# gau-nernst/pytorch-models

Measured on AMD Instinct MI355X. Metric: ViT-B/16 images/s & Whisper-base audio-sec/s (BASELINE.json metric; value / unit / ms_per_step = the ViT-B/16 leg of configs[1], the Whisper-base leg of configs[2] is the "whisper" object), higher is better.
Workload: dtype bf16; 1 GPU; ViT-B/16 bf16 forward, batch=256 per GPU, 224x224 (BASELINE configs[1]); per_gpu_batch=256, global_batch=256, parallelism=dp1, collective=none

## Files before the change

### include/pm_mi355x.h

```cpp
#ifndef PM_MI355X_H
#define PM_MI355X_H
#include <stdint.h>
#ifdef __cplusplus
extern "C" {
#endif

#define PM_ABI_VERSION 1

enum { PM_OK = 0, PM_EINVAL = 1, PM_EUNSUPPORTED = 2, PM_ELAUNCH = 3, PM_EALIGN = 4 };
enum { PM_BF16 = 0, PM_F32 = 1 };
enum { PM_ACT_NONE = 0, PM_ACT_GELU = 1, PM_ACT_GELU_TANH = 2, PM_ACT_RELU = 3, PM_ACT_SILU = 4 };

int pm_abi_version(void);
const char* pm_strerror(int code);

int pm_linear_bf16(const void* x, int64_t ldx, const void* w, int64_t ldw, const float* bias,
                   const void* resid, int64_t ldr, int resid_dtype, void* y, int64_t ldy, int y_dtype,
                   int64_t M, int64_t N, int64_t K, int act, void* stream);

int pm_linear_bf16_ex(const void* x, int64_t ldx, int64_t x_rows_per_batch, int64_t x_batch_stride, const void* w,
                      int64_t ldw, const float* bias, const void* resid, int64_t ldr, int resid_dtype,
                      int64_t resid_period, void* y, int64_t ldy, int y_dtype, int64_t M, int64_t N, int64_t K, int act,
                      void* stream);

// ... 195 lines not shown
                           int64_t k_stride_t, const void* v, int64_t v_stride_b, int64_t v_stride_t, void* o,
                           int64_t o_stride_b, int64_t o_stride_t, int64_t B, int64_t H, int64_t Lq, int64_t Lk, void* stream);

int pm_mixer_token_mix_bf16(const void* x, const float* stats, const float* gamma, const float* beta, const void* w1,
                            const float* b1, const void* w2, const float* b2, void* y, float* row_out, int64_t N, int64_t T,
                            int64_t Dt, int64_t C, void* stream);
int pm_mixer_token_mix_supported(int64_t T, int64_t Dt, int64_t C);

int pm_row_stats(const void* x, int64_t ldx, int x_dtype, float* stats, int64_t M, int64_t C, float eps, void* stream);

int pm_ln_mean(const void* x, int x_dtype, const float* stats, const float* gamma, const float* beta, void* y, int y_dtype,
               int64_t N, int64_t T, int64_t C, void* stream);

int pm_transpose_add_f32(const float* x, const float* resid, float* y, int64_t ldy, int64_t N, int64_t R, int64_t Cc, void* stream);

int pm_conv1d_f32(const float* x, int64_t x_batch_stride, const float* w, const float* bias, const float* resid, float* y,
                  int64_t B, int64_t Tin, int64_t Cin, int64_t Cout, int64_t k, int64_t stride, int64_t left, int64_t right,
                  int zero_pad, int elu, int64_t up, int64_t trim, int64_t Tout, void* stream);
int pm_conv1d_f32_supported(int64_t Tin, int64_t Cin, int64_t Cout, int64_t k, int64_t stride, int64_t left, int64_t right,
                            int zero_pad, int64_t up);

int pm_lstm_f32(const float* x, const float* const* w_ih, const float* const* w_hh, const float* const* bias, int64_t n_layers,
                float* work, float* y, int flags, int64_t B, int64_t T, int64_t H, void* stream);
int64_t pm_lstm_workspace_floats(int64_t B, int64_t T, int64_t H);

int pm_rvq_encode_f32(const float* z, const float* codebooks, const float* norms, int64_t* codes, int64_t M, int64_t n_q,
                      int64_t dim, int64_t codebook_size, void* stream);
int pm_rvq_decode_f32(const int64_t* codes, int64_t stride_b, int64_t stride_q, int64_t stride_t, const float* codebooks,
                      float* out, int64_t B, int64_t T, int64_t n_q, int64_t dim, int64_t codebook_size, void* stream);

int pm_groupnorm1_f32(float* x, const float* gamma, const float* beta, const float* resid, double* work, int64_t B, int64_t n,
                      int64_t C, float eps, void* stream);
int64_t pm_groupnorm1_workspace_doubles(int64_t B, int64_t n);

int pm_encodec_scale_f32(const float* x, float* scale, int64_t B, int64_t C, int64_t T, void* stream);
int pm_scale_clips_f32(const float* x, const float* scale, float* y, int64_t B, int64_t n, int divide, void* stream);

int pm_t5_dec_embed(const int64_t* tok, int64_t ldtok, const void* emb, float* x, int64_t B, int64_t d, int64_t V, void* stream);
int pm_t5_dec_self_fused(const float* x, int64_t d, const float* gamma, float eps, const void* w_qkv, void* kcache, void* vcache,
                         int64_t Tmax, const int32_t* pos_ptr, const float* lut, float* att, int64_t B, int64_t H, void* stream);
int pm_t5_dec_rms_qkv(const float* x, int64_t d, const float* gamma, float eps, const void* w_qkv, float* q, void* kcache,
                      void* vcache, int64_t Tmax, const int32_t* pos_ptr, int64_t B, int64_t H, void* stream);
int pm_t5_dec_self_attention(const float* q, const void* kcache, const void* vcache, int64_t Tmax, const int32_t* pos_ptr,
                             const float* lut, float* att, int64_t B, int64_t H, void* stream);
int pm_t5_dec_cross_fused(const float* x, int64_t d, const float* gamma, float eps, const void* w_q, const void* cross_kv,
                          int64_t S, const int32_t* src_len, float* att, int64_t B, int64_t H, void* stream);
int pm_t5_dec_geglu(const float* x, int64_t d, const float* gamma, float eps, const void* w_wv, float* h, int64_t ldh, int64_t B,
                    int64_t F, void* stream);
int pm_t5_dec_next_token(const float* ws_val, const int32_t* ws_idx, int64_t n_tiles, int32_t* pos_ptr, const int64_t* prompt,
                         int64_t P, int64_t* tokens, int64_t Ttot, int64_t pad_id, int64_t eos_id, int32_t* finished,
                         int64_t* out_lengths, const void* emb, float* x, int64_t d, int64_t V, int32_t* ticket,
                         const float* logits_step, float* logits_all, int64_t B, void* stream);

#ifdef __cplusplus
}
#endif
#endif
```

### pytorch-models_amd/pytorch_models/_hip/__init__.py

```python
from __future__ import annotations

import ctypes
import os
import re
from ctypes import c_char_p, c_float, c_int, c_int64, c_void_p

_HERE = os.path.dirname(os.path.abspath(__file__))
REPO_PKG_ROOT = os.path.dirname(os.path.dirname(_HERE))
LIB_PATH = os.environ.get("PM_MI355X_LIB") or os.path.join(REPO_PKG_ROOT, "csrc", "build", "libpm_mi355x.so")
HEADER_PATH = os.path.join(os.path.dirname(REPO_PKG_ROOT), "include", "pm_mi355x.h")

PM_BF16, PM_F32 = 0, 1
ACT = dict(none=0, gelu=1, approximate_gelu=2, relu=3, silu=4)

_p, _i, _l, _f = c_void_p, c_int, c_int64, c_float
SIGNATURES = {
    "pm_abi_version": ([], c_int),
    "pm_strerror": ([_i], c_char_p),
    "pm_linear_bf16": ([_p, _l, _p, _l, _p, _p, _l, _i, _p, _l, _i, _l, _l, _l, _i, _p], c_int),
    "pm_linear_bf16_ex": ([_p, _l, _l, _l, _p, _l, _p, _p, _l, _i, _l, _p, _l, _i, _l, _l, _l, _i, _p], c_int),
    "pm_linear_bf16_ln": ([_p, _l, _l, _l, _p, _l, _p, _p, _l, _i, _l, _p, _l, _i, _l, _l, _l, _i, _p, _p, _p, _p], c_int),
    "pm_linear_f32": ([_p, _l, _l, _l, _p, _l, _p, _p, _l, _l, _p, _l, _l, _l, _l, _i, _p], c_int),
    "pm_attention_generic_f32": ([_p, _l, _l, _p, _l, _l, _p, _l, _l, _p, _l, _l, _l, _l, _l, _l, _l, _i, _p, _l, _l, _l, _p], c_int),
    "pm_linear_bf16_ws": ([_p, _l, _l, _l, _p, _l, _p, _p, _l, _i, _l, _p, _l, _i, _l, _l, _l, _i, _p, _p, _p, _p, _l, _p], c_int),
# ... 22 lines not shown
    "pm_dec_whisper_rules": ([_p, _l, _l, _p, _l, _p, _l, _l, _l, _l, _l, _p, _l, _p, _l, _l, _p], c_int),
    "pm_dec_sample_topk": ([_p, _l, _l, _l, ctypes.c_uint64, _p, _p, _l, _p, _p, _l, _p, _p, _p, _l, _p, _l, _p], c_int),
    "pm_dec_next_token": ([_p, _p, _l, _p, _p, _l, _p, _p, _l, _p, _p, _p, _p, _l, _l, _p, _l, _p], c_int),
    "pm_layernorm": ([_p, _l, _i, _p, _p, _f, _p, _l, _i, _l, _l, _p], c_int),
    "pm_layernorm_ex": ([_p, _l, _i, _p, _p, _f, _i, _p, _l, _i, _p, _l, _i, _l, _l, _p], c_int),
    "pm_rmsnorm": ([_p, _l, _i, _p, _f, _p, _l, _i, _l, _l, _p], c_int),
    "pm_geglu": ([_p, _l, _p, _l, _l, _l, _p], c_int),
    "pm_w2v_stem0_scratch_floats": ([_l, _l], c_int64),
    "pm_w2v_stem0": ([_p, _p, _p, _i, _p, _p, _f, _p, _p, _p, _l, _l, _l, _l, _l, _p], c_int),
    "pm_group_windows": ([_p, _l, _i, _p, _l, _l, _l, _l, _l, _l, _l, _p], c_int),
    "pm_grouped_conv_supported": ([_l, _l], c_int),
    "pm_grouped_conv_bf16": ([_p, _p, _p, _p, _l, _p, _l, _l, _l, _l, _l, _l, _l, _l, _l, _i, _p], c_int),
    "pm_avgpool_time2": ([_p, _p, _l, _l, _l, _p], c_int),
    "pm_attention_bf16": ([_p, _l, _l, _p, _l, _l, _p, _l, _l, _p, _l, _l, _l, _l, _l, _l, _i, _p], c_int),
    "pm_attention_bias_bf16": ([_p, _l, _l, _p, _l, _l, _p, _l, _l, _p, _l, _l, _l, _l, _l, _l, _i, _p, _l, _l, _l, _p], c_int),
    "pm_attention_generic_bf16": ([_p, _l, _l, _p, _l, _l, _p, _l, _l, _p, _l, _l, _l, _l, _l, _l, _l, _i, _p, _l, _l, _l, _p], c_int),
    "pm_vit_tokens": ([_p, _p, _p, _p, _p, _p, _l, _l, _l, _l, _l, _p], c_int),
    "pm_vit_tokens_generic": ([_p, _p, _l, _p, _p, _p, _p, _l, _l, _l, _l, _l, _p], c_int),
    "pm_dwconv7_ln": ([_p, _i, _p, _p, _p, _p, _f, _p, _l, _i, _l, _l, _l, _l, _p], c_int),
    "pm_ln_space_to_depth": ([_p, _l, _i, _p, _p, _f, _p, _l, _i, _l, _l, _l, _l, _p], c_int),
    "pm_convnext_stem": ([_p, _p, _p, _p, _p, _f, _p, _l, _i, _l, _l, _l, _l, _p], c_int),
    "pm_mean_ln": ([_p, _l, _i, _p, _p, _f, _p, _i, _l, _l, _l, _p], c_int),
    "pm_window_attention_bf16": ([_p, _p, _p, _l, _p, _l, _p, _l, _l, _l, _l, _l, _i, _p], c_int),
    "pm_dwconv3_bn_act": ([_p, _i, _p, _p, _p, _p, _p, _p, _i, _l, _l, _l, _l, _i, _p], c_int),
    "pm_se_gate": ([_p, _l, _l, _p, _p, _p, _p, _p, _l, _l, _l, _p], c_int),
    "pm_maxvit_stem": ([_p, _p, _p, _p, _l, _i, _l, _l, _l, _l, _p], c_int),
    "pm_im2col3x3_nhwc": ([_p, _i, _p, _l, _i, _l, _l, _l, _l, _p], c_int),
    "pm_avgpool2x2_nhwc": ([_p, _i, _p, _i, _l, _l, _l, _l, _p], c_int),
    "pm_conv_bf16": ([_p, _l, _l, _l, _l, _p, _p, _p, _p, _l, _l, _l, _i, _p], c_int),
    "pm_resnet_stem": ([_p, _p, _p, _p, _p, _l, _l, _l, _p], c_int),
    "pm_attention_hd32_bf16": ([_p, _l, _l, _p, _l, _l, _p, _l, _l, _p, _l, _l, _l, _l, _l, _l, _p], c_int),
    "pm_mixer_token_mix_bf16": ([_p, _p, _p, _p, _p, _p, _p, _p, _p, _p, _l, _l, _l, _l, _p], c_int),
    "pm_mixer_token_mix_supported": ([_l, _l, _l], c_int),
    "pm_row_stats": ([_p, _l, _i, _p, _l, _l, _f, _p], c_int),
    "pm_ln_mean": ([_p, _i, _p, _p, _p, _p, _i, _l, _l, _l, _p], c_int),
    "pm_transpose_add_f32": ([_p, _p, _p, _l, _l, _l, _l, _p], c_int),
    "pm_conv1d_f32": ([_p, _l, _p, _p, _p, _p, _l, _l, _l, _l, _l, _l, _l, _l, _i, _i, _l, _l, _l, _p], c_int),
    "pm_conv1d_f32_supported": ([_l, _l, _l, _l, _l, _l, _l, _i, _l], c_int),
    "pm_lstm_f32": ([_p, _p, _p, _p, _l, _p, _p, _i, _l, _l, _l, _p], c_int),
    "pm_lstm_workspace_floats": ([_l, _l, _l], c_int64),
    "pm_rvq_encode_f32": ([_p, _p, _p, _p, _l, _l, _l, _l, _p], c_int),
    "pm_rvq_decode_f32": ([_p, _l, _l, _l, _p, _p, _l, _l, _l, _l, _l, _p], c_int),
    "pm_groupnorm1_f32": ([_p, _p, _p, _p, _p, _l, _l, _l, _f, _p], c_int),
    "pm_groupnorm1_workspace_doubles": ([_l, _l], c_int64),
    "pm_encodec_scale_f32": ([_p, _p, _l, _l, _l, _p], c_int),
    "pm_scale_clips_f32": ([_p, _p, _p, _l, _l, _i, _p], c_int),
    "pm_t5_dec_embed": ([_p, _l, _p, _p, _l, _l, _l, _p], c_int),
    "pm_t5_dec_self_fused": ([_p, _l, _p, _f, _p, _p, _p, _l, _p, _p, _p, _l, _l, _p], c_int),
    "pm_t5_dec_rms_qkv": ([_p, _l, _p, _f, _p, _p, _p, _p, _l, _p, _l, _l, _p], c_int),
    "pm_t5_dec_self_attention": ([_p, _p, _p, _l, _p, _p, _p, _l, _l, _p], c_int),
    "pm_t5_dec_cross_fused": ([_p, _l, _p, _f, _p, _p, _l, _p, _p, _l, _l, _p], c_int),
    "pm_t5_dec_geglu": ([_p, _l, _p, _f, _p, _p, _l, _l, _l, _p], c_int),
    "pm_t5_dec_next_token": ([_p, _p, _l, _p, _p, _l, _p, _l, _l, _l, _p, _p, _p, _p, _l, _l, _p, _p, _p, _l, _p], c_int),
}

EXPERIMENT_SIGNATURES = {
    "pm_dec_attention_fused_v2": ([_p, _l, _p, _p, _f, _p, _p, _p, _p, _l, _l, _l, _p, _l, _l, _p, _l, _l, _i, _p], c_int),
    "pm_dec_layers": ([_p, _l, _l, _l, _l, _l, _l, _l, _i, _l, _p, _p, _p, _p, _l, _p, _p, _p, _p, _p], c_int),
    "pm_dec_layers_grid": ([], c_int),
    "pm_gemm8ph_bench": ([_p, _l, _p, _l, _p, _l, _l, _l, _l, _p], c_int),
}


class DecLayer(ctypes.Structure):
    _fields_ = [(n, c_void_p) for n in (
        "sa_g", "sa_b", "w_qkv", "b_qkv", "kc", "vc", "w_so", "b_so", "ca_g", "ca_b", "w_q", "b_q", "cross_kv", "w_co", "b_co",
        "mlp_g", "mlp_b", "w1", "b1", "w2", "b2")] + [(n, c_float) for n in ("sa_eps", "ca_eps", "mlp_eps", "reserved_")]


_lib = None


def header_functions() -> list[str]:
    src = open(HEADER_PATH).read()
    src = re.sub(r"/\*.*?\*/", "", src, flags=re.S)
    return sorted(set(re.findall(r"\b(pm_[a-z0-9_]+)\s*\(", src)))


def lib() -> ctypes.CDLL:
    global _lib
    if _lib is None:
        if not os.path.exists(LIB_PATH):
            raise RuntimeError(
                f"{LIB_PATH} is missing: the MI355X HIP library has not been built "
                "(run `make -C pytorch-models_amd/csrc` or `python -c 'import __graft_entry__ as g; g.build()'`). "
                "This package has no CPU or eager fallback."
            )
        L = ctypes.CDLL(LIB_PATH)
        for name, (argtypes, restype) in SIGNATURES.items():
            fn = getattr(L, name)
            fn.argtypes = argtypes
            fn.restype = restype
        for name, (argtypes, restype) in EXPERIMENT_SIGNATURES.items():
            if hasattr(L, name):
                fn = getattr(L, name)
                fn.argtypes = argtypes
                fn.restype = restype
        if L.pm_abi_version() != 1:
            raise RuntimeError(f"libpm_mi355x ABI {L.pm_abi_version()} != binding ABI 1: rebuild the library")
        _lib = L
    return _lib


def has_experiments() -> bool:
    return hasattr(lib(), "pm_dec_layers")

# ... 5 lines not shown
```

### pytorch-models_amd/pytorch_models/_hip/ops.py

```python
from __future__ import annotations

import os

import torch
from torch import Tensor

from . import ACT, PM_BF16, PM_F32, check, lib


_raw_stream = getattr(torch._C, "_cuda_getCurrentRawStream", None)
_cur_device = getattr(torch._C, "_cuda_getDevice", None)


def _stream() -> int:
    if _raw_stream is not None and _cur_device is not None:
        return _raw_stream(_cur_device())
    return torch.cuda.current_stream().cuda_stream


def _current_device_index() -> int:
    return _cur_device() if _cur_device is not None else torch.cuda.current_device()


def check_devices(*ts) -> None:
# ... 1009 lines not shown
    _f32c(codebooks, "rvq_decode: codebooks")
    B, n_q, T = codes.shape
    Q, N, D = codebooks.shape
    _need(1 <= n_q <= Q, f"rvq_decode: {n_q} code streams for {Q} codebooks")
    out = torch.empty((B, T, D), dtype=torch.float32, device=codes.device)
    rc = _launch("rvq_decode_f32", (0.0, float(out.numel() * 4 * (n_q + 1))), lambda: lib().pm_rvq_decode_f32(
        codes.data_ptr(), codes.stride(0), codes.stride(1), codes.stride(2), codebooks.data_ptr(), out.data_ptr(), B, T, n_q, D, N, _stream()))
    check(rc, f"pm_rvq_decode_f32(B={B}, T={T}, n_q={n_q})")
    return out


def groupnorm1_(x: Tensor, gamma: Tensor, beta: Tensor, eps: float, resid: Tensor | None = None) -> Tensor:
    _cuda(x, gamma, beta, resid)
    _need(x.dim() == 3, "groupnorm1_: x must be (B, T, C)")
    _f32c(x, "groupnorm1_: x")
    B, T, C = x.shape
    _f32vec(gamma, C, "groupnorm1_: gamma")
    _f32vec(beta, C, "groupnorm1_: beta")
    if resid is not None:
        _need(resid.shape == x.shape, "groupnorm1_: resid must have x's shape")
        _f32c(resid, "groupnorm1_: resid")
    _need(B <= 65535 and T >= 1, "groupnorm1_: at most 65535 clips, at least one frame")
    work = torch.empty((lib().pm_groupnorm1_workspace_doubles(B, T * C),), dtype=torch.float64, device=x.device)
    rc = _launch("groupnorm1_f32", (0.0, float(x.numel() * 12)), lambda: lib().pm_groupnorm1_f32(
        x.data_ptr(), gamma.data_ptr(), beta.data_ptr(), resid.data_ptr() if resid is not None else None, work.data_ptr(), B, T * C, C,
        float(eps), _stream()))
    check(rc, f"pm_groupnorm1_f32(B={B}, T={T}, C={C})")
    return x


def encodec_scale(x: Tensor) -> Tensor:
    _cuda(x)
    _need(x.dim() == 3, "encodec_scale: x must be (B, C, T)")
    _f32c(x, "encodec_scale: x")
    B, C, T = x.shape
    _need(T >= 1 and C >= 1, "encodec_scale: empty clip")
    out = torch.empty((B, 1, 1), dtype=torch.float32, device=x.device)
    rc = _launch("encodec_scale_f32", (0.0, float(x.numel() * 4)), lambda: lib().pm_encodec_scale_f32(x.data_ptr(), out.data_ptr(), B, C, T, _stream()))
    check(rc, f"pm_encodec_scale_f32(B={B}, C={C}, T={T})")
    return out


def scale_clips(x: Tensor, scale: Tensor, divide: bool) -> Tensor:
    _cuda(x, scale)
    _f32c(x, "scale_clips: x")
    _f32c(scale, "scale_clips: scale")
    B = x.shape[0]
    _need(x.dim() >= 2 and scale.numel() == B and B <= 65535 and x.numel() > 0, "scale_clips: one scale per clip, at most 65535 clips")
    out = torch.empty_like(x)
    rc = _launch("scale_clips_f32", (0.0, float(x.numel() * 8)), lambda: lib().pm_scale_clips_f32(
        x.data_ptr(), scale.data_ptr(), out.data_ptr(), B, x.numel() // B, int(divide), _stream()))
    check(rc, "pm_scale_clips_f32")
    return out
```

### pytorch-models_amd/pytorch_models/image/vit.py

```python
from __future__ import annotations

from functools import partial

import torch
import torch.nn.functional as F
from torch import Tensor, nn

from .. import _cpu
from .._hip import ops
from ..transformer import MHA, MLP, Encoder, LayerNorm, _f32, _fused_mlp, _wb, derived


class ClassTokenPooling(nn.Module):
    def forward(self, x: Tensor) -> Tensor:
        return x[:, 0]


class GlobalAveragePooling(nn.Module):
    def forward(self, x: Tensor) -> Tensor:
        return x.mean(1)


class MHAPooling(nn.Module):

# ... 30 lines not shown
        super().__init__()
        self.patch_embed = nn.Conv2d(3, d_model, patch_size, patch_size)
        self.cls_token = nn.Parameter(torch.zeros(1, 1, d_model)) if cls_token else None
        self.pe = nn.Parameter(torch.zeros(1, (img_size // patch_size) ** 2, d_model))
        self.layers = Encoder(n_layers, d_model, n_heads=n_heads, dropout=dropout, norm_eps=self.norm_eps)
        self.layers.pm_streams = 2
        self.norm = LayerNorm(d_model, self.norm_eps)
        poolers = dict(
            cls_token=ClassTokenPooling,
            gap=GlobalAveragePooling,
            mha=partial(MHAPooling, d_model, n_heads, norm_eps=self.norm_eps),
        )
        self.pooler = poolers[pool_type]()

    def tokens(self, imgs: Tensor) -> Tensor:
        if _cpu.on_cpu(imgs, self.patch_embed.weight):
            return _cpu.vit_tokens(self, imgs)
        if self.patch_embed.weight.dtype == torch.float32:
            return self._tokens_f32(imgs)
        pw = self.patch_embed.weight
        if pw.shape[2] == 16:
            w2d = pw.view(pw.shape[0], -1)
        else:
            def pad():
                k = 3 * pw.shape[2] * pw.shape[3]
                w = torch.zeros(pw.shape[0], (k + 63) // 64 * 64, dtype=pw.dtype, device=pw.device)
                w[:, :k] = pw.detach().reshape(pw.shape[0], -1)
                return w

            w2d = derived(self, "w2d_pad", (pw,), pad)
        cls = None if self.cls_token is None else _f32(self, "cls", self.cls_token).view(-1)
        return ops.vit_tokens(imgs.float().contiguous(), w2d, _f32(self, "pb", self.patch_embed.bias),
                              _f32(self, "pe", self.pe).view(-1, pw.shape[0]), cls, pw.shape[2])

    def _tokens_f32(self, imgs: Tensor) -> Tensor:
        w = self.patch_embed.weight
        d, _, P, _ = w.shape
        N, _, H, W = imgs.shape
        gh, gw = H // P, W // P
        cols = imgs.float().unfold(2, P, P).unfold(3, P, P).permute(0, 2, 3, 1, 4, 5).reshape(N * gh * gw, 3 * P * P)
        pe = self.pe.float().view(-1, d)
        if pe.shape[0] != gh * gw:
            raise ValueError(f"ViT: pe holds {pe.shape[0]} positions, the image has {gh * gw} patches; call resize_pe first")
        y = ops.linear_f32(cols, w.view(d, -1), self.patch_embed.bias, resid=pe.contiguous(), resid_period=gh * gw).view(N, gh * gw, d)
        if self.cls_token is not None:
            y = torch.cat([self.cls_token.float().expand(N, 1, d), y], 1)
        return y

    def forward(self, imgs: Tensor) -> Tensor:
        n_tok = self.pe.shape[1] + (self.cls_token is not None)
        parts = None
        if imgs.dim() == 4 and imgs.is_cuda and self.patch_embed.weight.dtype == torch.bfloat16:
            parts = self.layers.split_sizes(imgs.shape[0], n_tok, torch.bfloat16, imgs.device)
        if parts is None:
            out = self.layers(self.tokens(imgs))
        else:
            out = self.layers(producers=[lambda lo=lo, hi=hi: self.tokens(imgs[lo:hi]) for lo, hi in parts], device=imgs.device)
        io = self.patch_embed.weight.dtype
        if isinstance(self.pooler, ClassTokenPooling):
            return self.norm(out[:, 0], io)
        if out.device.type == "cpu":
            return self.pooler(self.norm(out))
        return self.pooler(self.norm(out)).to(io)

    @torch.no_grad()
    def resize_pe(self, size: int, interpolation_mode: str = "bicubic") -> None:
        g_old = int(self.pe.shape[1] ** 0.5)
        g_new = size // self.patch_embed.weight.shape[2]
        grid = self.pe.float().unflatten(1, (g_old, g_old)).permute(0, 3, 1, 2)
        grid = F.interpolate(grid, (g_new, g_new), mode=interpolation_mode)
        self.pe = nn.Parameter(grid.permute(0, 2, 3, 1).flatten(1, 2).to(self.pe.dtype))

    def load_flax_ckpt(self, ckpt, *, big_vision: bool = False, prefix: str = "") -> None:
        from ..converters import load_flax_vit

        left = load_flax_vit(self, ckpt, big_vision=big_vision, prefix=prefix)
        if left:
            print(left)

    def load_facebook_state_dict(self, state_dict) -> None:
        from ..converters import load_facebook_vit

        print(load_facebook_vit(self, state_dict))

    @staticmethod
    def _parse(model_tag: str, default_weights: str):
        tag, weights = model_tag.split("_") if "_" in model_tag else (model_tag, default_weights)
        size, patch = tag.split("/")
        return tag, weights, _SIZES[size], int(patch)

    @staticmethod
    def from_google(model_tag: str, *, pretrained: bool = False, **kwargs) -> "ViT":
        _, weights, (n_layers, d_model, n_heads), patch = ViT._parse(model_tag, "augreg")
        extra = dict(cls_token=False, pool_type="mha") if weights == "siglip" else {}
        m = ViT(n_layers, d_model, n_heads, patch, **extra, **kwargs)
        if pretrained:
            if weights not in ("augreg", "siglip"):
                raise ValueError(f"Unsupported weights={weights}")
            _no_download("ViT.from_google")
        return m

    @staticmethod
    def from_facebook(model_tag: str, *, pretrained: bool = False, **kwargs) -> "ViT":
        _, weights, (n_layers, d_model, n_heads), patch = ViT._parse(model_tag, "deit3")
        if weights in ("deit3", "dino"):
            kwargs.setdefault("img_size", 224)
        elif weights == "dinov2":
            kwargs.setdefault("img_size", 518)
        else:
            raise ValueError(f"Unsupported {weights}")
        m = ViT(n_layers, d_model, n_heads, patch, **kwargs)
        if pretrained:
            _no_download("ViT.from_facebook")
# ... 26 lines not shown
```

### pytorch-models_amd/pytorch_models/transformer.py

```python
from __future__ import annotations

import os

import torch
from torch import Tensor, nn

from . import _cpu
from ._hip import ops

_ACTS = {
    "gelu": lambda: nn.GELU(),
    "approximate_gelu": lambda: nn.GELU(approximate="tanh"),
    "relu": lambda: nn.ReLU(inplace=True),
    "silu": lambda: nn.SiLU(),
}


def _sig(ts) -> tuple:
    return tuple((t.data_ptr(), 0 if t.is_inference() else t._version, t.dtype, t.device) for t in ts if t is not None)


def derived(module: nn.Module, key: str, params, build):
    store = module.__dict__.setdefault("_pm_derived", {})
    sig = _sig(params)
# ... 89 lines not shown
        return y.view(*x.shape[:-1], self.out_features)


class MHA(nn.Module):
    def __init__(
        self,
        d_model: int,
        n_heads: int | None = None,
        head_dim: int | None = None,
        bias: bool = True,
        dropout: float = 0.0,
    ) -> None:
        if n_heads is None and head_dim is None:
            head_dim = 64
        if head_dim is None:
            head_dim = d_model // n_heads
        if n_heads is None:
            n_heads = d_model // head_dim
        super().__init__()
        inner = n_heads * head_dim
        self.q_proj = Linear(d_model, inner, bias)
        self.k_proj = Linear(d_model, inner, bias)
        self.v_proj = Linear(d_model, inner, bias)
        self.out_proj = Linear(inner, d_model, bias)
        self.n_heads = n_heads
        self.head_dim = head_dim
        self.dropout = dropout

    def _pack(self, names: str):
        mods = [getattr(self, f"{n}_proj") for n in names]
        params = [m.weight for m in mods] + [m.bias for m in mods]

        def build():
            w = torch.cat([m.weight.detach() for m in mods], 0).to(torch.bfloat16).contiguous()
            b = None if mods[0].bias is None else torch.cat([m.bias.detach().float() for m in mods], 0).contiguous()
            return w, b

        return derived(self, "pack_" + names, params, build)

    def _pack32(self, names: str):
        mods = [getattr(self, f"{n}_proj") for n in names]
        params = [m.weight for m in mods] + [m.bias for m in mods]

        def build():
            w = torch.cat([m.weight.detach().float() for m in mods], 0).contiguous()
            b = None if mods[0].bias is None else torch.cat([m.bias.detach().float() for m in mods], 0).contiguous()
            return w, b

        return derived(self, "pack32_" + names, params, build)

    def _pack_ln(self, norm: "LayerNorm"):
        w, b = self._pack("qkv")
        return derived(self, "pack_qkv_ln", (w, b, norm.weight, norm.bias), lambda: _fold_ln(w, b, norm))

    def forward(
        self,
        q: Tensor,
        k: Tensor | None = None,
        v: Tensor | None = None,
        attn_bias: Tensor | None = None,
        causal: bool = False,
    ) -> Tensor:
        return self.attend(q, k, v, attn_bias, causal)

    def attend(self, q, k=None, v=None, attn_bias=None, causal=False, residual: Tensor | None = None) -> Tensor:
        if _cpu.on_cpu(q, self.q_proj.weight):
            return _cpu.mha(self, q, k, v, attn_bias, causal, residual)
        _require_bf16(q, self.q_proj.weight, "MHA")
        if self.head_dim % 2 or self.head_dim > 128 or (self.head_dim % 4 and self.head_dim > 64):
            raise NotImplementedError(f"MHA: head_dim {self.head_dim} is not covered by the gfx950 attention kernels (% 4 up to 128, % 2 up to 64)")
        if self.training and self.dropout > 0.0:
            raise NotImplementedError("MHA: inference only (attention dropout is not implemented)")
        H, inner = self.n_heads, self.n_heads * self.head_dim
        Lq = q.shape[-2]
        if _is32(self.q_proj.weight):
            return self._attend_f32(q, k, v, attn_bias, causal, residual)
        io_dtype = q.dtype
        q = _xb(q)
        k = None if k is None else _xb(k)
        v = None if v is None else _xb(v)
        if k is None and v is None:
            lead = q.shape[:-2]
            w, b = self._pack("qkv")
            qkv = ops.linear(q.reshape(-1, q.shape[-1]), w, b).view(-1, Lq, 3 * inner)
            qh, kh, vh = qkv[..., :inner], qkv[..., inner : 2 * inner], qkv[..., 2 * inner :]
        else:
            k = q if k is None else k
            Lk = k.shape[-2]
            lead = torch.broadcast_shapes(q.shape[:-2], k.shape[:-2])
            qh = self.q_proj(q)
            if v is None or v is k:
                w, b = self._pack("kv")
                kv = ops.linear(k.reshape(-1, k.shape[-1]), w, b).view(*k.shape[:-1], 2 * inner)
                kh, vh = kv[..., :inner], kv[..., inner:]
            else:
                kh, vh = self.k_proj(k), self.v_proj(v)
            qh = qh.expand(*lead, Lq, inner).reshape(-1, Lq, inner)
            kh = kh.expand(*lead, Lk, inner).reshape(-1, Lk, inner)
            vh = vh.expand(*lead, Lk, inner).reshape(-1, Lk, inner)
        bias4 = None if attn_bias is None else _bias4(attn_bias, lead, Lq, kh.shape[1])
        o = ops.attention(qh, kh, vh, H, causal, bias4)
        res2 = None if residual is None else residual.reshape(-1, residual.shape[-1])
        y = ops.linear(o.view(-1, inner), _wb(self.out_proj, "w", self.out_proj.weight), _f32(self.out_proj, "b", self.out_proj.bias),
                       resid=res2, out_dtype=io_dtype)
        return y.view(*lead, Lq, y.shape[-1])

# ... 151 lines not shown
        n_heads: int | None = None,
        head_dim: int | None = None,
        bias: bool = True,
        mlp_ratio: float = 4.0,
        dropout: float = 0.0,
        act: str = "gelu",
        pre_norm: bool = True,
        norm_eps: float = 1e-5,
    ) -> None:
        super().__init__(d_model, n_heads, head_dim, False, bias, mlp_ratio, dropout, act, pre_norm, norm_eps)

    def forward(self, x: Tensor) -> Tensor:
        return DecoderLayer.forward(self, x, None)

    def chain_ok(self, x: Tensor) -> bool:
        sa, mlp = self.sa, self.mlp
        if not (self.pre_norm and type(sa).forward is MHA.forward and type(mlp).forward is MLP.forward and x.is_cuda
                and x.dtype == torch.bfloat16 and sa.q_proj.weight.dtype == torch.bfloat16 and not self.training):
            return False
        M, d = x.numel() // x.shape[-1], x.shape[-1]
        inner, hid = sa.n_heads * sa.head_dim, mlp.linear1.out_features
        if sa.head_dim % 8 or sa.head_dim > 128 or mlp.act_name not in ("gelu",):
            return False
        return (ops.linear_ln_supported(M, d, inner, "none", True) and ops.linear_ln_supported(M, d, hid, "none", True)
                and ops.linear_ln_supported(M, 3 * inner, d, "none", False)
                and ops.linear_ln_supported(M, hid, d, mlp.act_name, False))

    def forward_chain(self, x: Tensor, stats: Tensor | None, next_eps: float | None):
        sa, mlp = self.sa, self.mlp
        lead, d = x.shape[:-1], x.shape[-1]
        H, inner = sa.n_heads, sa.n_heads * sa.head_dim
        x2 = x.reshape(-1, d)
        if stats is None:
            w, b = sa._pack("qkv")
            qkv = ops.linear(self.sa_norm(x2), w, b)
        else:
            wl, s, c = sa._pack_ln(self.sa_norm)
            qkv = ops.linear(x2, wl, c, ln_stats=stats, ln_s=s)
        qkv = qkv.view(-1, x.shape[-2], 3 * inner)
        o = ops.attention(qkv[..., :inner], qkv[..., inner : 2 * inner], qkv[..., 2 * inner :], H, False, None)
        x2, rows = ops.linear(o.view(-1, inner), sa.out_proj.weight, _f32(sa.out_proj, "b", sa.out_proj.bias), resid=x2,
                              want_row_stats=True)
        st = ops.ln_stats_finalize(rows, d, self.mlp_norm.eps)
        l1, l2 = mlp.linear1, mlp.linear2
        wl, s, c = derived(mlp, "l1_ln", (l1.weight, l1.bias, self.mlp_norm.weight, self.mlp_norm.bias),
                           lambda: _fold_ln(l1.weight, l1.bias, self.mlp_norm))
        h = ops.linear(x2, wl, c, act=mlp.act_name, ln_stats=st, ln_s=s)
        if next_eps is None:
            return ops.linear(h, l2.weight, _f32(l2, "b", l2.bias), resid=x2).view(*lead, d), None
        x2, rows = ops.linear(h, l2.weight, _f32(l2, "b", l2.bias), resid=x2, want_row_stats=True)
        return x2.view(*lead, d), ops.ln_stats_finalize(rows, d, next_eps)


class Encoder(nn.Sequential):
    def __init__(
        self,
        n_layers: int,
        d_model: int,
        n_heads: int | None = None,
        head_dim: int | None = None,
        bias: bool = True,
        mlp_ratio: float = 4.0,
        dropout: float = 0.0,
        act: str = "gelu",
        pre_norm: bool = True,
        norm_eps: float = 1e-5,
    ) -> None:
        super().__init__(*[
            EncoderLayer(d_model, n_heads, head_dim, bias, mlp_ratio, dropout, act, pre_norm, norm_eps)
            for _ in range(n_layers)
        ])

    def forward(self, x: Tensor | None = None, *, producers=None, device: torch.device | None = None) -> Tensor:
        layers = list(self)
        fold = os.environ.get("PM_LN_FOLD", "1") != "0"

        def plan(t: Tensor):
            return [fold and isinstance(l, EncoderLayer) and type(l).forward is EncoderLayer.forward and l.chain_ok(t) for l in layers]

        def step(i: int, ok, t: Tensor, stats):
            if not ok[i]:
                return layers[i](t), None
            nxt = layers[i + 1].sa_norm.eps if i + 1 < len(layers) and ok[i + 1] else None
            return layers[i].forward_chain(t, stats, nxt)

        halves = self._two_streams(x) if producers is None else None
        if halves is not None and any(plan(h) != plan(halves[0]) for h in halves[1:]):
            halves = None
        if halves is None and producers is None:
            ok, stats = plan(x), None
            for i in range(len(layers)):
                x, stats = step(i, ok, x, stats)
            return x
        n_parts = len(halves) if producers is None else len(producers)
        device = halves[0].device if producers is None else device
        cur = torch.cuda.current_stream(device)
        streams = [cur] + [_side_stream(device, k) for k in range(1, n_parts)]
        out = None
        if producers is None:
            out = torch.empty_like(x)
        elif getattr(self, "_pm_out_shape", None) is not None:
            shape, dtype = self._pm_out_shape
            out = torch.empty(shape, dtype=dtype, device=device)
        for st in streams[1:]:
            st.wait_stream(cur)
        if producers is None:
            state = [(h, None) for h in halves]
        else:
            state = []
            for k in range(n_parts):
                with torch.cuda.stream(streams[k]):
                    state.append((producers[k](), None))
        oks = [plan(t) for t, _ in state]
        first = [0]
        for t, _ in state:
            first.append(first[-1] + t.shape[0])
        want = ((first[-1],) + tuple(state[0][0].shape[1:]), state[0][0].dtype)
        if out is None or (tuple(out.shape), out.dtype) != want:
            out = torch.empty(want[0], dtype=want[1], device=device)
            for st in streams[1:]:
                st.wait_stream(cur)
        if producers is not None:
            self._pm_out_shape = want
        if any(o != oks[0] for o in oks[1:]):
            for k in range(n_parts):
                with torch.cuda.stream(streams[k]):
                    out[first[k] : first[k + 1]].copy_(state[k][0])
            for st in streams[1:]:
                cur.wait_stream(st)
            return self.forward(out)
        for i in range(len(layers)):
            for k in reversed(range(n_parts)):
                with torch.cuda.stream(streams[k]):
                    state[k] = step(i, oks[k], state[k][0], state[k][1])
                    if i == len(layers) - 1:
                        out[first[k] : first[k + 1]].copy_(state[k][0])
                        state[k] = None
        for st in streams[1:]:
            cur.wait_stream(st)
        return out

    def split_sizes(self, batch: int, tokens: int, dtype: torch.dtype, device: torch.device):
        want = ENCODER_STREAMS or int(os.environ.get("PM_ENCODER_STREAMS", "0")) or self.pm_streams
        if want < 2 or device.type != "cuda" or batch < 2 or dtype != torch.bfloat16 or batch * tokens < _MIN_SPLIT_ROWS:
            return None
        want = min(want, 4, batch)
        cuts = [batch * k // want for k in range(want + 1)]
        return [(cuts[k], cuts[k + 1]) for k in range(want)]

    pm_streams = 1

    def _two_streams(self, x: Tensor):
        if x.dim() != 3:
            return None
        cuts = self.split_sizes(x.shape[0], x.shape[1], x.dtype, x.device)
        return None if cuts is None else [x[lo:hi] for lo, hi in cuts]


class Decoder(nn.ModuleList):
    def __init__(
        self,
        n_layers: int,
        d_model: int,
        n_heads: int | None = None,
        head_dim: int | None = None,
        cross_attn: bool = False,
        bias: bool = True,
        mlp_ratio: float = 4.0,
        dropout: float = 0.0,
        act: str = "gelu",
        pre_norm: bool = True,
        norm_eps: float = 1e-5,
    ) -> None:
        super().__init__([
            DecoderLayer(d_model, n_heads, head_dim, cross_attn, bias, mlp_ratio, dropout, act, pre_norm, norm_eps)
            for _ in range(n_layers)
        ])

    def forward(self, x: Tensor, memory: Tensor | None = None) -> Tensor:
        for layer in self:
            x = layer(x, memory)
        return x
```

Measured before the change: 27460 images/s.

## Compute only the CLS row in the final ViT encoder layer

When the pooler uses the class token, the last encoder layer now evaluates only row 0. It computes the CLS query, folds the LayerNorm into the K/V projections per head, and runs a fused HIP kernel that attends the CLS query over all tokens using raw activations and LN stats. The MLP and out-projection then run on a single row per image instead of 197. This removes about 1/12 of the encoder work, at the cost of new kernels, extra plumbing through the multi-stream path, and a different numerical path through the folded LayerNorm.

```diff
diff --git a/include/pm_mi355x.h b/include/pm_mi355x.h
--- a/include/pm_mi355x.h
+++ b/include/pm_mi355x.h
@@ -271,6 +271,12 @@
                          int64_t* out_lengths, const void* emb, float* x, int64_t d, int64_t V, int32_t* ticket,
                          const float* logits_step, float* logits_all, int64_t B, void* stream);
 
+int pm_cls_attend(const void* x, int64_t x_row_stride, int64_t x_batch_stride, const float* stats, const void* u, void* ctx,
+                  int64_t N, int64_t L, int64_t d, int64_t H, float scale, float eps, void* stream);
+int pm_cls_attend_supported(int64_t L, int64_t d, int64_t H);
+int pm_cls_head_gemm(const void* x, int64_t ldx, int64_t x_group_stride, const void* w, const float* bias, void* y, int64_t ldy,
+                     int64_t y_group_stride, int64_t M, int64_t N, int64_t K, int64_t G, void* stream);
+
 #ifdef __cplusplus
 }
 #endif
diff --git a/pytorch-models_amd/csrc/cls_tail.hip b/pytorch-models_amd/csrc/cls_tail.hip
--- /dev/null
+++ b/pytorch-models_amd/csrc/cls_tail.hip
@@ -0,0 +1,298 @@
+#include "common.h"
+
+namespace {
+
+constexpr int CT_JB = 32;
+constexpr int CT_THREADS = 256;
+constexpr int CT_MAX_D = 1024;
+constexpr int CT_SIDE_BYTES = 4 * 16 * CT_JB * 4 + 16 * CT_JB * 2 + CT_JB * 2 * 4 + 16 * 4 + 4 * 16 * 4 + 16 * 2 * 4;
+
+__device__ __forceinline__ void ct_glds16(const void* gsrc, unsigned lds_dst_wave_base) {
+  unsigned keep;
+  const unsigned dst = __builtin_amdgcn_readfirstlane(lds_dst_wave_base);
+  asm volatile("s_mov_b32 %0, m0\n\ts_mov_b32 m0, %2\n\ts_nop 0\n\tglobal_load_lds_dwordx4 %1, off\n\ts_mov_b32 m0, %0"
+               : "=&s"(keep)
+               : "v"(gsrc), "s"(dst)
+               : "memory");
+}
+
+__device__ __forceinline__ bf16x8 ct_tr_pair(const unsigned char* p0, const unsigned char* p1) {
+  union { s16x4 h[2]; bf16x8 v; } u;
+  u.h[0] = __builtin_amdgcn_ds_read_tr16_b64_v4i16((PM_LDS s16x4*)p0);
+  u.h[1] = __builtin_amdgcn_ds_read_tr16_b64_v4i16((PM_LDS s16x4*)p1);
+  return u.v;
+}
+
+__device__ __forceinline__ float sum16(float v) {
+#pragma unroll
+  for (int o = 1; o < 16; o <<= 1) v += __shfl_xor(v, o, 64);
+  return v;
+}
+__device__ __forceinline__ float max16(float v) {
+#pragma unroll
+  for (int o = 1; o < 16; o <<= 1) v = fmaxf(v, __shfl_xor(v, o, 64));
+  return v;
+}
+
+__global__ __launch_bounds__(CT_THREADS) void cls_attend_kernel(const bf16* __restrict__ x, int64_t x_rs, int64_t x_bs,
+                                                                const float* __restrict__ stats, const bf16* __restrict__ u,
+                                                                bf16* __restrict__ ctx, int L, int d, int H, float scale, float eps) {
+  extern __shared__ __attribute__((aligned(16))) unsigned char smem[];
+  const int tid = threadIdx.x, lane = tid & 63, fr = lane & 15, fq = lane >> 4;
+  const int wv = __builtin_amdgcn_readfirstlane(tid >> 6);
+  const int n = blockIdx.x;
+  const int P = d >> 6, nks = d >> 5, nct = d >> 4;
+  const int XB = 64 * d;
+  float* sc = (float*)(smem + 2 * XB);
+  bf16* wt = (bf16*)(sc + 4 * 16 * CT_JB);
+  float* st = (float*)(wt + 16 * CT_JB);
+  float* al = st + CT_JB * 2;
+  float* su = al + 16;
+  float* fin = su + 4 * 16;
+  const unsigned lds0 = (unsigned)(uintptr_t)(PM_LDS unsigned char*)smem;
+  const bf16* xn = x + (int64_t)n * x_bs;
+  const int nblk = (L + CT_JB - 1) / CT_JB;
+
+  auto stage = [&](int b) {
+    const unsigned buf = lds0 + (b & 1) * XB;
+    for (int pc = wv; pc < 4 * P; pc += 4) {
+      const int p = pc >> 2, rg = pc & 3;
+      const int r = rg * 8 + (lane >> 3), c = swz_pos(r, lane & 7);
+      const int j = min(b * CT_JB + r, L - 1);
+      ct_glds16(xn + (int64_t)j * x_rs + p * 64 + c * 8, buf + p * 4096 + rg * 1024);
+    }
+  };
+  f32x2 stn = {0.f, 1.f};
+  if (stats && tid < CT_JB) stn = *(const f32x2*)(stats + ((int64_t)n * L + min(tid, L - 1)) * 2);
+  stage(0);
+
+  bf16x8 uf[8];
+  {
+    const bf16* up = u + ((int64_t)n * H + min(fr, H - 1)) * d + fq * 8;
+    float s = 0.f;
+#pragma unroll
+    for (int t = 0; t < 8; ++t) {
+      const int ks = wv + 4 * t;
+      bf16x8 v = *(const bf16x8*)(up + min(ks, nks - 1) * 32);
+      if (ks >= nks || fr >= H)
+#pragma unroll
+        for (int e = 0; e < 8; ++e) v[e] = (bf16)0.0f;
+      uf[t] = v;
+#pragma unroll
+      for (int e = 0; e < 8; ++e) s += (float)v[e];
+    }
+    s += __shfl_xor(s, 16, 64);
+    s += __shfl_xor(s, 32, 64);
+    if (fq == 0) su[wv * 16 + fr] = s;
+  }
+
+  f32x4 acc[16];
+#pragma unroll
+  for (int t = 0; t < 16; ++t) acc[t] = f32x4{0.f, 0.f, 0.f, 0.f};
+  const int sh = tid >> 4, sj = tid & 15;
+  float m_run = -INFINITY, l_run = 0.f, cm_run = 0.f, su_h = 0.f;
+
+  for (int b = 0; b < nblk; ++b) {
+    const unsigned char* buf = smem + (b & 1) * XB;
+    const int j0 = b * CT_JB;
+    asm volatile("s_waitcnt vmcnt(0)" ::: "memory");
+    __syncthreads();
+    if (stats && tid < CT_JB) {
+      *(f32x2*)(st + 2 * tid) = stn;
+      if (b + 1 < nblk) stn = *(const f32x2*)(stats + ((int64_t)n * L + min(j0 + CT_JB + tid, L - 1)) * 2);
+    }
+    if (b + 1 < nblk) stage(b + 1);
+    if (b == 0) su_h = su[sh] + su[16 + sh] + su[32 + sh] + su[48 + sh];
+
+    if (!stats) {
+      for (int rr = 0; rr < 8; ++rr) {
+        const int r = wv * 8 + rr;
+        float s = 0.f;
+        for (int c = lane; c < d / 8; c += 64) {
+          const bf16x8 v = *(const bf16x8*)(buf + (c >> 3) * 4096 + r * 128 + swz_pos(r, c & 7) * 16);
+#pragma unroll
+          for (int e = 0; e < 8; ++e) s += (float)v[e];
+        }
+        const float mean = wave_sum(s) / (float)d;
+        float q = 0.f;
+        for (int c = lane; c < d / 8; c += 64) {
+          const bf16x8 v = *(const bf16x8*)(buf + (c >> 3) * 4096 + r * 128 + swz_pos(r, c & 7) * 16);
+#pragma unroll
+          for (int e = 0; e < 8; ++e) {
+            const float dv = (float)v[e] - mean;
+            q = fmaf(dv, dv, q);
+          }
+        }
+        const float var = wave_sum(q) / (float)d;
+        if (lane == 0) {
+          st[2 * r] = mean;
+          st[2 * r + 1] = rsqrtf(var + eps);
+        }
+      }
+    }
+
+    {
+      f32x4 sa[2] = {f32x4{0.f, 0.f, 0.f, 0.f}, f32x4{0.f, 0.f, 0.f, 0.f}};
+#pragma unroll
+      for (int t = 0; t < 8; ++t) {
+        const int ks = wv + 4 * t;
+        if (ks < nks) {
+          const unsigned char* pb = buf + (ks >> 1) * 4096;
+          const int ch = (ks & 1) * 4 + fq;
+#pragma unroll
+          for (int jt = 0; jt < 2; ++jt) {
+            const int row = jt * 16 + fr;
+            const bf16x8 bx = *(const bf16x8*)(pb + row * 128 + swz_pos(row, ch) * 16);
+            sa[jt] = __builtin_amdgcn_mfma_f32_16x16x32_bf16(uf[t], bx, sa[jt], 0, 0, 0);
+          }
+        }
+      }
+#pragma unroll
+      for (int jt = 0; jt < 2; ++jt)
+#pragma unroll
+        for (int i = 0; i < 4; ++i) sc[(wv * 16 + fq * 4 + i) * CT_JB + jt * 16 + fr] = sa[jt][i];
+    }
+    __syncthreads();
+
+    {
+      float s[2], mean[2], rstd[2];
+#pragma unroll
+      for (int r = 0; r < 2; ++r) {
+        const int j = sj + 16 * r;
+        const float dot = ((sc[sh * CT_JB + j] + sc[(16 + sh) * CT_JB + j]) + sc[(32 + sh) * CT_JB + j]) + sc[(48 + sh) * CT_JB + j];
+        mean[r] = st[2 * j];
+        rstd[r] = st[2 * j + 1];
+        s[r] = j0 + j < L ? scale * rstd[r] * (dot - mean[r] * su_h) : -INFINITY;
+      }
+      const float m_new = fmaxf(m_run, max16(fmaxf(s[0], s[1])));
+      const float alpha = __expf(m_run - m_new);
+      const float p0 = __expf(s[0] - m_new), p1 = __expf(s[1] - m_new);
+      const bf16 w0 = (bf16)(p0 * rstd[0]), w1 = (bf16)(p1 * rstd[1]);
+      l_run = fmaf(l_run, alpha, sum16(p0 + p1));
+      cm_run = fmaf(cm_run, alpha, sum16(fmaf((float)w0, mean[0], (float)w1 * mean[1])));
+      m_run = m_new;
+      wt[sh * CT_JB + sj] = w0;
+      wt[sh * CT_JB + sj + 16] = w1;
+      if (sj == 0) al[sh] = alpha;
+    }
+    __syncthreads();
+
+    {
+      const bf16x8 wf = *(const bf16x8*)(wt + fr * CT_JB + fq * 8);
+      const float a = al[fr];
+      const int q = fr >> 2, p = fr & 3;
+      const int r0 = 8 * fq + q, r1 = r0 + 4;
+#pragma unroll
+      for (int t = 0; t < 16; ++t) {
+        const int ct = wv + 4 * t;
+        if (ct < nct) {
+          const unsigned char* pb = buf + (ct >> 2) * 4096;
+          const int ch = (ct & 3) * 2 + (p >> 1);
+          const bf16x8 xf = ct_tr_pair(pb + r0 * 128 + swz_pos(r0, ch) * 16 + (p & 1) * 8,
+                                       pb + r1 * 128 + swz_pos(r1, ch) * 16 + (p & 1) * 8);
+          acc[t] = __builtin_amdgcn_mfma_f32_16x16x32_bf16(xf, wf, acc[t] * a, 0, 0, 0);
+        }
+      }
+    }
+  }
+
+  if (sj == 0) {
+    fin[2 * sh] = cm_run;
+    fin[2 * sh + 1] = l_run;
+  }
+  __syncthreads();
+  if (fr < H) {
+    const float cm = fin[2 * fr], inv = 1.0f / fin[2 * fr + 1];
+    bf16* cp = ctx + ((int64_t)n * H + fr) * d + fq * 4;
+#pragma unroll
+    for (int t = 0; t < 16; ++t) {
+      const int ct = wv + 4 * t;
+      if (ct < nct) {
+        bf16x4 o;
+#pragma unroll
+        for (int i = 0; i < 4; ++i) o[i] = (bf16)((acc[t][i] - cm) * inv);
+        *(bf16x4*)(cp + ct * 16) = o;
+      }
+    }
+  }
+}
+
+__global__ __launch_bounds__(256) void cls_head_gemm_kernel(const bf16* __restrict__ x, int64_t ldx, int64_t xg,
+                                                            const bf16* __restrict__ w, const float* __restrict__ bias,
+                                                            bf16* __restrict__ y, int64_t ldy, int64_t yg, int M, int N, int K) {
+  __shared__ __attribute__((aligned(16))) float red[4][16][68];
+  const int tid = threadIdx.x, lane = tid & 63, fr = lane & 15, fq = lane >> 4;
+  const int wv = __builtin_amdgcn_readfirstlane(tid >> 6);
+  const int m0 = blockIdx.x * 16, n0 = blockIdx.y * 64, g = blockIdx.z;
+  const bf16* xp = x + (int64_t)min(m0 + fr, M - 1) * ldx + (int64_t)g * xg + fq * 8;
+  const bf16* wp = w + ((int64_t)g * N + n0 + fr) * K + fq * 8;
+  f32x4 acc[4];
+#pragma unroll
+  for (int j = 0; j < 4; ++j) acc[j] = f32x4{0.f, 0.f, 0.f, 0.f};
+  const int nks = K >> 5;
+  for (int ks = wv; ks < nks; ks += 4) {
+    const bf16x8 b = *(const bf16x8*)(xp + ks * 32);
+    bf16x8 a[4];
+#pragma unroll
+    for (int j = 0; j < 4; ++j) a[j] = *(const bf16x8*)(wp + (int64_t)j * 16 * K + ks * 32);
+#pragma unroll
+    for (int j = 0; j < 4; ++j) acc[j] = __builtin_amdgcn_mfma_f32_16x16x32_bf16(a[j], b, acc[j], 0, 0, 0);
+  }
+#pragma unroll
+  for (int j = 0; j < 4; ++j) *(f32x4*)&red[wv][fr][j * 16 + fq * 4] = acc[j];
+  __syncthreads();
+  const int row = tid >> 4, c4 = (tid & 15) * 4;
+  if (m0 + row < M) {
+    f32x4 v = ((*(const f32x4*)&red[0][row][c4] + *(const f32x4*)&red[1][row][c4]) + *(const f32x4*)&red[2][row][c4]) +
+              *(const f32x4*)&red[3][row][c4];
+    if (bias) v += *(const f32x4*)(bias + (int64_t)g * N + n0 + c4);
+    bf16x4 o;
+#pragma unroll
+    for (int i = 0; i < 4; ++i) o[i] = (bf16)v[i];
+    *(bf16x4*)(y + (int64_t)(m0 + row) * ldy + (int64_t)g * yg + n0 + c4) = o;
+  }
+}
+
+inline bool ct_al(const void* p, uintptr_t a) { return ((uintptr_t)p & (a - 1)) == 0; }
+
+}
+
+extern "C" int pm_cls_attend_supported(int64_t L, int64_t d, int64_t H) {
+  return L >= 1 && L <= (1 << 20) && d >= 64 && d % 64 == 0 && d <= CT_MAX_D && H >= 1 && H <= 16 ? 1 : 0;
+}
+
+extern "C" int pm_cls_attend(const void* x, int64_t x_row_stride, int64_t x_batch_stride, const float* stats, const void* u,
+                             void* ctx, int64_t N, int64_t L, int64_t d, int64_t H, float scale, float eps, void* stream) {
+  if (!x || !u || !ctx || N < 0 || L < 1 || d < 64 || d % 64 || H < 1 || H > 16 || x_row_stride < d) return PM_EINVAL;
+  if (d > CT_MAX_D || L > (1 << 20) || N > 0x7fffffff) return PM_EUNSUPPORTED;
+  if (!ct_al(x, 16) || !ct_al(u, 16) || !ct_al(ctx, 8) || !ct_al(stats, 8) || x_row_stride % 8 || x_batch_stride % 8) return PM_EALIGN;
+  if (N == 0) return PM_OK;
+  const size_t lds = (size_t)(2 * 64 * d + CT_SIDE_BYTES);
+  if (lds > 64 * 1024) {
+    static bool raised = false;
+    if (!raised) {
+      if (hipFuncSetAttribute((const void*)cls_attend_kernel, hipFuncAttributeMaxDynamicSharedMemorySize, 2 * 64 * CT_MAX_D + CT_SIDE_BYTES) !=
+          hipSuccess)
+        return PM_ELAUNCH;
+      raised = true;
+    }
+  }
+  hipLaunchKernelGGL(cls_attend_kernel, dim3((unsigned)N), dim3(CT_THREADS), lds, (hipStream_t)stream, (const bf16*)x, x_row_stride,
+                     x_batch_stride, stats, (const bf16*)u, (bf16*)ctx, (int)L, (int)d, (int)H, scale, eps);
+  PM_CHECK_LAUNCH();
+  return PM_OK;
+}
+
+extern "C" int pm_cls_head_gemm(const void* x, int64_t ldx, int64_t x_group_stride, const void* w, const float* bias, void* y,
+                                int64_t ldy, int64_t y_group_stride, int64_t M, int64_t N, int64_t K, int64_t G, void* stream) {
+  if (!x || !w || !y || M < 0 || N < 64 || N % 64 || K < 32 || K % 32 || G < 1) return PM_EINVAL;
+  if (G > 65535 || N / 64 > 65535 || M > (1 << 24) || K > (1 << 20)) return PM_EUNSUPPORTED;
+  if (!ct_al(x, 16) || !ct_al(w, 16) || !ct_al(y, 8) || !ct_al(bias, 16) || ldx % 8 || x_group_stride % 8 || ldy % 4 || y_group_stride % 4)
+    return PM_EALIGN;
+  if (M == 0) return PM_OK;
+  const dim3 grid((unsigned)((M + 15) / 16), (unsigned)(N / 64), (unsigned)G);
+  hipLaunchKernelGGL(cls_head_gemm_kernel, grid, dim3(256), 0, (hipStream_t)stream, (const bf16*)x, ldx, x_group_stride, (const bf16*)w,
+                     bias, (bf16*)y, ldy, y_group_stride, (int)M, (int)N, (int)K);
+  PM_CHECK_LAUNCH();
+  return PM_OK;
+}
diff --git a/pytorch-models_amd/pytorch_models/_hip/__init__.py b/pytorch-models_amd/pytorch_models/_hip/__init__.py
--- a/pytorch-models_amd/pytorch_models/_hip/__init__.py
+++ b/pytorch-models_amd/pytorch_models/_hip/__init__.py
@@ -98,6 +98,9 @@
     "pm_t5_dec_cross_fused": ([_p, _l, _p, _f, _p, _p, _l, _p, _p, _l, _l, _p], c_int),
     "pm_t5_dec_geglu": ([_p, _l, _p, _f, _p, _p, _l, _l, _l, _p], c_int),
     "pm_t5_dec_next_token": ([_p, _p, _l, _p, _p, _l, _p, _l, _l, _l, _p, _p, _p, _p, _l, _l, _p, _p, _p, _l, _p], c_int),
+    "pm_cls_attend": ([_p, _l, _l, _p, _p, _p, _l, _l, _l, _l, _f, _f, _p], c_int),
+    "pm_cls_attend_supported": ([_l, _l, _l], c_int),
+    "pm_cls_head_gemm": ([_p, _l, _l, _p, _p, _p, _l, _l, _l, _l, _l, _l, _p], c_int),
 }
 
 EXPERIMENT_SIGNATURES = {
diff --git a/pytorch-models_amd/pytorch_models/_hip/ops.py b/pytorch-models_amd/pytorch_models/_hip/ops.py
--- a/pytorch-models_amd/pytorch_models/_hip/ops.py
+++ b/pytorch-models_amd/pytorch_models/_hip/ops.py
@@ -1085,3 +1085,40 @@
         x.data_ptr(), scale.data_ptr(), out.data_ptr(), B, x.numel() // B, int(divide), _stream()))
     check(rc, "pm_scale_clips_f32")
     return out
+
+
+def cls_attend_supported(L: int, d: int, H: int) -> bool:
+    return bool(lib().pm_cls_attend_supported(L, d, H))
+
+
+def cls_head_gemm(x: Tensor, w: Tensor, bias: Tensor | None = None) -> Tensor:
+    _cuda(x, w, bias)
+    G, N, K = w.shape
+    _need(x.dtype == torch.bfloat16 and w.dtype == torch.bfloat16 and w.is_contiguous(), "cls_head_gemm: bf16 x, contiguous bf16 w (G, N, K)")
+    M = x.shape[0]
+    x2 = x.reshape(M, G * K)
+    _need(x2.stride(1) == 1, "cls_head_gemm: x rows must be contiguous")
+    if bias is not None:
+        _need(bias.dtype == torch.float32 and bias.is_contiguous() and bias.numel() == G * N, "cls_head_gemm: bias must be f32 (G * N)")
+    out = torch.empty((M, G, N), dtype=torch.bfloat16, device=x.device)
+    rc = _launch("cls_head_gemm", (2.0 * M * G * N * K, float(2 * (x2.numel() + w.numel() + out.numel()))), lambda: lib().pm_cls_head_gemm(
+        x2.data_ptr(), x2.stride(0), K, w.data_ptr(), bias.data_ptr() if bias is not None else None, out.data_ptr(), G * N, N,
+        M, N, K, G, _stream()))
+    check(rc, f"pm_cls_head_gemm(M={M}, N={N}, K={K}, G={G})")
+    return out
+
+
+def cls_attend(x: Tensor, stats: Tensor | None, u: Tensor, scale: float, eps: float) -> Tensor:
+    _cuda(x, stats, u)
+    _need(x.dim() == 3 and u.dim() == 3 and x.dtype == torch.bfloat16 and u.dtype == torch.bfloat16 and x.stride(2) == 1
+          and u.is_contiguous() and u.shape[0] == x.shape[0] and u.shape[2] == x.shape[2], "cls_attend: x (N, L, d), u (N, H, d) bf16")
+    N, L, d = x.shape
+    H = u.shape[1]
+    if stats is not None:
+        _need(stats.dtype == torch.float32 and stats.is_contiguous() and stats.shape == (N * L, 2), "cls_attend: stats must be f32 (N*L, 2)")
+    out = torch.empty((N, H, d), dtype=torch.bfloat16, device=x.device)
+    rc = _launch("cls_attend", (4.0 * N * H * L * d, float(2 * (x.numel() + 2 * u.numel()))), lambda: lib().pm_cls_attend(
+        x.data_ptr(), x.stride(1), x.stride(0), stats.data_ptr() if stats is not None else None, u.data_ptr(), out.data_ptr(),
+        N, L, d, H, float(scale), float(eps), _stream()))
+    check(rc, f"pm_cls_attend(N={N}, L={L}, d={d}, H={H})")
+    return out
diff --git a/pytorch-models_amd/pytorch_models/image/vit.py b/pytorch-models_amd/pytorch_models/image/vit.py
--- a/pytorch-models_amd/pytorch_models/image/vit.py
+++ b/pytorch-models_amd/pytorch_models/image/vit.py
@@ -106,13 +106,15 @@
         parts = None
         if imgs.dim() == 4 and imgs.is_cuda and self.patch_embed.weight.dtype == torch.bfloat16:
             parts = self.layers.split_sizes(imgs.shape[0], n_tok, torch.bfloat16, imgs.device)
+        cls = isinstance(self.pooler, ClassTokenPooling)
         if parts is None:
-            out = self.layers(self.tokens(imgs))
+            out = self.layers(self.tokens(imgs), first_row=cls)
         else:
-            out = self.layers(producers=[lambda lo=lo, hi=hi: self.tokens(imgs[lo:hi]) for lo, hi in parts], device=imgs.device)
+            out = self.layers(producers=[lambda lo=lo, hi=hi: self.tokens(imgs[lo:hi]) for lo, hi in parts], device=imgs.device,
+                              first_row=cls)
         io = self.patch_embed.weight.dtype
-        if isinstance(self.pooler, ClassTokenPooling):
-            return self.norm(out[:, 0], io)
+        if cls:
+            return self.norm(out, io)
         if out.device.type == "cpu":
             return self.pooler(self.norm(out))
         return self.pooler(self.norm(out)).to(io)
diff --git a/pytorch-models_amd/pytorch_models/transformer.py b/pytorch-models_amd/pytorch_models/transformer.py
--- a/pytorch-models_amd/pytorch_models/transformer.py
+++ b/pytorch-models_amd/pytorch_models/transformer.py
@@ -165,6 +165,18 @@
     def _pack_ln(self, norm: "LayerNorm"):
         w, b = self._pack("qkv")
         return derived(self, "pack_qkv_ln", (w, b, norm.weight, norm.bias), lambda: _fold_ln(w, b, norm))
+
+    def _pack_cls(self, norm: "LayerNorm"):
+        kp, vp = self.k_proj, self.v_proj
+
+        def build():
+            H, hd = self.n_heads, self.head_dim
+            wkl, _, _ = _fold_ln(kp.weight, None, norm)
+            wvl, _, cv = _fold_ln(vp.weight, vp.bias, norm)
+            d = wkl.shape[1]
+            return wkl.view(H, hd, d).transpose(1, 2).contiguous(), wvl.view(H, hd, d).contiguous(), cv
+
+        return derived(self, "pack_cls", (kp.weight, vp.weight, vp.bias, norm.weight, norm.bias), build)
 
     def forward(
         self,
@@ -422,6 +434,37 @@
         return x2.view(*lead, d), ops.ln_stats_finalize(rows, d, next_eps)
 
 
+    def first_row_ok(self, x: Tensor) -> bool:
+        sa, mlp = self.sa, self.mlp
+        if os.environ.get("PM_VIT_CLS_TAIL", "1") == "0":
+            return False
+        if not (type(self).forward is EncoderLayer.forward and self.pre_norm and type(sa).forward is MHA.forward
+                and type(sa).attend is MHA.attend and type(mlp).forward is MLP.forward and type(mlp).run is MLP.run
+                and type(self.sa_norm) is LayerNorm and type(self.mlp_norm) is LayerNorm and not self.training):
+            return False
+        if not (x.dim() == 3 and x.is_cuda and x.dtype == torch.bfloat16 and x.stride(2) == 1 and x.shape[1] >= 1
+                and sa.q_proj.weight.is_cuda and sa.q_proj.weight.dtype == torch.bfloat16
+                and mlp.linear1.weight.dtype == torch.bfloat16):
+            return False
+        d = x.shape[2]
+        return (sa.head_dim == 64 and sa.q_proj.in_features == d and sa.k_proj.in_features == d and sa.v_proj.in_features == d
+                and x.stride(1) % 8 == 0 and x.stride(0) % 8 == 0 and ops.cls_attend_supported(x.shape[1], d, sa.n_heads))
+
+    def forward_first_row(self, x: Tensor, stats: Tensor | None, out: Tensor | None = None) -> Tensor:
+        sa, mlp = self.sa, self.mlp
+        B, d = x.shape[0], x.shape[2]
+        x0 = x[:, 0]
+        q = ops.linear(self.sa_norm(x0), sa.q_proj.weight, _f32(sa.q_proj, "b", sa.q_proj.bias))
+        wku, wvh, cv = sa._pack_cls(self.sa_norm)
+        u = ops.cls_head_gemm(q, wku)
+        ctx = ops.cls_attend(x, stats, u, sa.head_dim ** -0.5, self.sa_norm.eps)
+        o = ops.cls_head_gemm(ctx, wvh, cv).view(B, -1)
+        y = ops.linear(o, sa.out_proj.weight, _f32(sa.out_proj, "b", sa.out_proj.bias), resid=x0)
+        l1, l2 = mlp.linear1, mlp.linear2
+        h = ops.linear(self.mlp_norm(y), l1.weight, _f32(l1, "b", l1.bias), act=mlp.act_name)
+        return ops.linear(h, l2.weight, _f32(l2, "b", l2.bias), resid=y, out=out)
+
+
 class Encoder(nn.Sequential):
     def __init__(
         self,
@@ -441,7 +484,8 @@
             for _ in range(n_layers)
         ])
 
-    def forward(self, x: Tensor | None = None, *, producers=None, device: torch.device | None = None) -> Tensor:
+    def forward(self, x: Tensor | None = None, *, producers=None, device: torch.device | None = None,
+                first_row: bool = False) -> Tensor:
         layers = list(self)
         fold = os.environ.get("PM_LN_FOLD", "1") != "0"
 
@@ -459,16 +503,20 @@
             halves = None
         if halves is None and producers is None:
             ok, stats = plan(x), None
-            for i in range(len(layers)):
+            tail = first_row and bool(layers) and isinstance(layers[-1], EncoderLayer) and layers[-1].first_row_ok(x)
+            for i in range(len(layers) - tail):
                 x, stats = step(i, ok, x, stats)
-            return x
+            if tail:
+                return layers[-1].forward_first_row(x, stats)
+            return x[:, 0] if first_row else x
         n_parts = len(halves) if producers is None else len(producers)
         device = halves[0].device if producers is None else device
         cur = torch.cuda.current_stream(device)
         streams = [cur] + [_side_stream(device, k) for k in range(1, n_parts)]
         out = None
+        tail = first_row and producers is None and bool(layers) and isinstance(layers[-1], EncoderLayer) and all(layers[-1].first_row_ok(h) for h in halves)
         if producers is None:
-            out = torch.empty_like(x)
+            out = x.new_empty((x.shape[0], x.shape[2])) if tail else torch.empty_like(x)
         elif getattr(self, "_pm_out_shape", None) is not None:
             shape, dtype = self._pm_out_shape
             out = torch.empty(shape, dtype=dtype, device=device)
@@ -485,30 +533,37 @@
         first = [0]
         for t, _ in state:
             first.append(first[-1] + t.shape[0])
-        want = ((first[-1],) + tuple(state[0][0].shape[1:]), state[0][0].dtype)
+        mixed = any(o != oks[0] for o in oks[1:])
+        if producers is not None:
+            tail = first_row and not mixed and bool(layers) and isinstance(layers[-1], EncoderLayer) and all(layers[-1].first_row_ok(t) for t, _ in state)
+        want = ((first[-1],) + tuple(state[0][0].shape[2 if tail else 1:]), state[0][0].dtype)
         if out is None or (tuple(out.shape), out.dtype) != want:
             out = torch.empty(want[0], dtype=want[1], device=device)
             for st in streams[1:]:
                 st.wait_stream(cur)
         if producers is not None:
             self._pm_out_shape = want
-        if any(o != oks[0] for o in oks[1:]):
+        if mixed:
             for k in range(n_parts):
                 with torch.cuda.stream(streams[k]):
                     out[first[k] : first[k + 1]].copy_(state[k][0])
             for st in streams[1:]:
                 cur.wait_stream(st)
-            return self.forward(out)
+            return self.forward(out, first_row=first_row)
         for i in range(len(layers)):
             for k in reversed(range(n_parts)):
                 with torch.cuda.stream(streams[k]):
+                    if tail and i == len(layers) - 1:
+                        layers[i].forward_first_row(state[k][0], state[k][1], out=out[first[k] : first[k + 1]])
+                        state[k] = None
+                        continue
                     state[k] = step(i, oks[k], state[k][0], state[k][1])
                     if i == len(layers) - 1:
                         out[first[k] : first[k + 1]].copy_(state[k][0])
                         state[k] = None
         for st in streams[1:]:
             cur.wait_stream(st)
-        return out
+        return out[:, 0] if first_row and not tail else out
 
     def split_sizes(self, batch: int, tokens: int, dtype: torch.dtype, device: torch.device):
         want = ENCODER_STREAMS or int(os.environ.get("PM_ENCODER_STREAMS", "0")) or self.pm_streams
```

After: 29270 images/s, median of 6. +6.6%, better.
